# matsui528/rii

Measured on AMD Instinct MI355X. Metric: queries/sec, higher is better.
Workload: dtype f32; 1 GPU; SIFT1M-shaped linear search, D=128 M=32 Ks=256, N=1000000, batch=1024 per GPU, topk=1; global_batch=1024, lut_mode=exact, simd_order=avx512, scan_mode=8-bit filter + exact fp32 re-rank

## Files before the change

rii_amd/csrc/engine.hip:

```cpp
#include "rii_amd.h"
#include "rii_internal.h"

#include <algorithm>
#include <chrono>
#include <cmath>
#include <cstdarg>
#include <cstdio>
#include <cstring>
#include <map>
#include <mutex>
#include <numeric>
#include <random>
#include <string>
#include <thread>
#include <vector>

#define RII_API extern "C" __attribute__((visibility("default")))

using namespace riiamd;

static thread_local std::string g_err;
static int set_err(int code, const char *fmt, ...)
{
    char buf[1024];
// ... 133 lines not shown
    int timing = 0;
    hipStream_t stream = nullptr;
    int n_cu = 256;

    std::vector<float> codewords;
    std::vector<uint8_t> codes;
    std::vector<uint8_t> centers;
    std::vector<std::vector<int32_t>> lists;
    int64_t N = 0;

    DevBuf d_codewords, d_cnorm, d_codes, d_centers, d_symtab, d_pl_off, d_pl_ids, d_list_len;
    DevBuf d_lcodes; bool lcodes_valid = false;
    bool lcodes_failed = false, rot_failed = false;
    DevBuf d_rcent, d_rlcodes, d_rl_toff; bool rot_valid = false;
    int64_t quad_launches = 0;
    int64_t rot_launches = 0;
    DevBuf d_scan_codes, d_scan_perm;
    DevBuf d_fcodes;

    int64_t fc_cov = 0;
    int scan_order = 1;
    int scan_mx = 1;
    int slice_topk = 1;
    int host_spin = 1;
    bool ivf_q_host = false;
    unsigned int *spin_flag = nullptr;
    unsigned int spin_seq = 0;
    bool spin_used = false;
    int64_t spin_nflags = 0;
    int host_zero_copy = 1;
    int fused_rerank = 0;
    int small_topk = 1;
    int scan_pipe = 1;
    int scan_dual = 1;
    int64_t scan_cov = 0;
    int64_t scan_N = -1;
    bool have_symtab = false, have_cnorm = false, lists_dirty = true;


    std::map<std::string, KernelTimer> timers;
    std::vector<hipEvent_t> event_pool;

    ScratchSet parked;
    int lanes = 2;
    mutable std::mutex mu;

};

namespace {

int64_t nlist_of(const rii_engine *e) { return e->M ? (int64_t) (e->centers.size() / (size_t) e->M) : 0; }

bool timer_wanted(const rii_engine *e, const char *name)
{
    if (e->timing == 1) return true;
    if (e->timing == 2) return !strcmp(name, "scan") || !strcmp(name, "ivf_fused") || !strcmp(name, "ivf_scan") || !strcmp(name, "ivf_shard") || !strcmp(name, "shard_coarse");
    return false;
}
hipEvent_t timer_event(rii_engine *e)
{
    if (!e->event_pool.empty()) {
        hipEvent_t ev = e->event_pool.back();
        e->event_pool.pop_back();
        return ev;
    }
    hipEvent_t ev = nullptr;
// ... 268 lines not shown
        }
        HIP_TRY(launch_lut_build_mfma(d_queries, B, e->d_codewords.as<float>(), e->d_cnorm.as<float>(), e->M, e->Ks,
                                      e->Ds, qt, e->s_lut.as<float>(), st));
    } else {
        HIP_TRY(launch_lut_build(d_queries, B, e->d_codewords.as<float>(), e->M, e->Ks, e->Ds, e->arch, qt,
                                 e->s_lut.as<float>(), st));
    }
    return RII_OK;
}

int exact_tile_for(const rii_engine *e, int64_t B, int topk) { return (topk == 1 && B <= 2 && e->QT >= (int) B) ? (int) B : e->QT; }

void pick_chunks(const rii_engine *e, int64_t n_codes, int64_t B, int *chunks, int64_t *chunk_len, int qt = 0)
{
    if (qt <= 0) qt = e->QT;
    const int64_t tiles = (B + qt - 1) / qt;
    int64_t c = e->scan_chunks;
    if (c <= 0) {
        const bool stream_form = qt <= 2 && (size_t) qt * e->M * e->Ks * sizeof(float) <= ((size_t) 64 << 10);
        const int64_t target = (stream_form ? 4LL : 2LL) * e->n_cu;
        c = (target + tiles - 1) / tiles;
        const int64_t max_c = std::max<int64_t>(1, n_codes / 8192);
        c = std::max<int64_t>(1, std::min(c, max_c));
        if (tiles >= e->n_cu) c = 1;
    }
    c = std::max<int64_t>(1, std::min<int64_t>(c, 65535));
    int64_t len = (n_codes + c - 1) / c;
    len = std::max<int64_t>(len, 1);
    *chunks = (int) ((n_codes + len - 1) / len);
    *chunk_len = len;
}

constexpr int64_t kScanOrderMinN = 1 << 16;

int ensure_scan_order(rii_engine *e, hipStream_t st)
{
    if (e->scan_N == e->N) return RII_OK;
    const size_t M = (size_t) e->M;
    const int64_t cov = std::min(e->scan_cov, e->N);
    RII_TRY(e->d_scan_codes.ensure((size_t) e->N * M, (size_t) cov * M, st));
    RII_TRY(e->d_scan_perm.ensure((size_t) e->N * sizeof(int32_t), (size_t) cov * sizeof(int32_t), st));
    {
        ScopedTimer t(e, "scan_order", st);
        HIP_TRY(launch_scan_order(e->d_codes.as<uint8_t>(), e->N, e->M, e->Ks, fastscan_rows(e->M, e->Ks), cov / 1024,
                                  e->d_scan_perm.as<int32_t>(),
                                  e->d_scan_codes.as<uint8_t>(), st));
    }
    e->scan_cov = (e->N / 1024) * 1024;
    e->scan_N = e->N;
    HIP_TRY(hipStreamSynchronize(st));
    return RII_OK;
}

int ensure_fcodes(rii_engine *e, hipStream_t st)
{
    if (e->fc_cov == e->N) return RII_OK;
    RII_TRY(e->d_fcodes.ensure((size_t) fcodes_bytes(e->N, e->M, e->scan_mx), (size_t) fcodes_bytes(e->fc_cov, e->M, e->scan_mx), st));
    {
        ScopedTimer t(e, "format", st);
        HIP_TRY(launch_fcodes_format(e->d_codes.as<uint8_t>(), nullptr, e->fc_cov, e->N, e->M, e->Ks, e->d_fcodes.as<uint16_t>(),
                                     e->scan_mx, st));
    }
    e->fc_cov = e->N;
    HIP_TRY(hipStreamSynchronize(st));
    return RII_OK;
}
// ... 150 lines not shown
            if (!e->qlut_ready) {
                ScopedTimer t(e, "quant", st);
                RII_TRY(e->s_qc.ensure((size_t) B * e->M * e->Ks));
                const int lv = generic_table_levels(e);
                HIP_TRY(launch_lut_quantize(e->s_lut.as<float>(), B, e->M, e->Ks, e->lut_qt, e->s_qc.as<uint8_t>(),
                                            e->s_qlut.as<uint8_t>(), e->s_slack.as<int32_t>(), e->scan_mx, st, lv));
                e->qlut_levels = lv;
            }
            if (!e->qlut_ready) HIP_TRY(hipMemsetAsync(e->s_cand_cnt.p, 0, (size_t) B * sizeof(unsigned int), st));
            e->last_fs_B = B;
            if (topk == 1) {
                RII_TRY(e->s_gthr.ensure((size_t) B * sizeof(uint32_t)));
                if (!e->qlut_ready)
                    HIP_TRY(hipMemsetAsync(e->s_gthr.p, 0xff, (size_t) B * sizeof(uint32_t), st));
                const bool tail_rr = !e->lut_valid && e->fused_rerank && !d_perm && fscan_tail_supported(e->M, e->Ks, e->Ds, e->scan_mx);
                FsTail tl;
                if (tail_rr) {
                    RII_TRY(ensure_tile_done(e, st));
                    tl.queries = d_queries; tl.codewords = e->d_codewords.as<float>(); tl.codes = d_rr; tl.remap = d_remap;
                    tl.indirect = indirect; tl.Ds = e->Ds; tl.topk = topk; tl.out_ids = d_out_ids; tl.out_dists = d_out_dists;
                    tl.tile_done = e->s_tile_done.as<unsigned int>();
                    const int64_t nfl = fscan_tail_flags(e->M, e->Ks, e->scan_mx, e->scan_dual, B);
                    if (e->spin_flag && nfl * sizeof(unsigned int) <= kPinFlagWords * sizeof(unsigned int)) {
                        tl.host_flag = e->spin_flag; tl.seq = e->spin_seq;
                        e->spin_used = true; e->spin_nflags = nfl;
                    }
                }
                {
                    ScopedTimer t(e, "scan", st, true);
                    HIP_TRY(launch_fscan(d_scan, n_codes, e->M, e->Ks, e->s_qlut.as<uint8_t>(), e->s_slack.as<int32_t>(),
                                         (int) B, chunks, len, e->s_cand.as<unsigned long long>(),
                                         e->s_cand_cnt.as<unsigned int>(), cap, 0, nullptr, nullptr,
                                         e->s_gthr.as<uint32_t>(), 1, e->scan_mx, st, e->qlut_quarter ? 1 : 0, e->scan_dual, e->qlut_levels,
                                         tail_rr ? &tl : nullptr, e->scan_pipe == 2 || (e->scan_pipe == 1 && B <= 128)));
                }
                if (tail_rr) return RII_OK;
                ScopedTimer t(e, "rerank", st);
                if (!e->lut_valid) {
                    HIP_TRY(launch_rerank_top1_direct(d_rr, n_codes, e->M, e->Ds, d_queries, e->d_codewords.as<float>(),
                                                      e->s_slack.as<int32_t>(), e->s_cand.as<unsigned long long>(),
                                                      e->s_cand_cnt.as<unsigned int>(), cap, d_remap, B, d_out_ids, d_out_dists, topk,
                                                      indirect, st));
                    return RII_OK;
                }
                HIP_TRY(launch_rerank_top1(d_rr, n_codes, e->M, e->Ks, e->s_lut.as<float>(), e->lut_qt,
                                           e->s_slack.as<int32_t>(), e->s_cand.as<unsigned long long>(),
                                           e->s_cand_cnt.as<unsigned int>(), cap, d_remap, d_perm, B, d_out_ids, d_out_dists, topk,
                                           indirect, st, e->d_cand_peak.as<unsigned int>()));
                if (e->h_cand_peak && e->d_cand_peak.p)
                    HIP_TRY(hipMemcpyAsync(e->h_cand_peak, e->d_cand_peak.p, sizeof(unsigned int), hipMemcpyDeviceToHost, st));
                return RII_OK;
            }
            RII_TRY(e->s_segmin.ensure((size_t) B * G * sizeof(uint16_t)));
            RII_TRY(e->s_thr16.ensure((size_t) B * sizeof(uint32_t)));
            {
                ScopedTimer t(e, "scan", st, true);
                HIP_TRY(launch_fscan(d_scan, n_codes, e->M, e->Ks, e->s_qlut.as<uint8_t>(), e->s_slack.as<int32_t>(), (int) B,
                                     chunks, len, nullptr, nullptr, 0, 1, e->s_segmin.as<uint16_t>(), nullptr, nullptr, stride,
                                     e->scan_mx, st, e->qlut_quarter ? 1 : 0, e->scan_dual, e->qlut_levels));
            }
            {
                ScopedTimer t(e, "kth", st);
                HIP_TRY(launch_kth_threshold(e->s_segmin.as<uint16_t>(), G, B, topk, fastscan_max_sum(e->M, e->qlut_levels),
                                             e->s_slack.as<int32_t>(), e->s_thr16.as<uint32_t>(), st));
            }
            {
                ScopedTimer t(e, "scan", st, true);
// ... 1957 lines not shown
        e->shard_pre = (int) value;
    } else if (k == "ivf_quad") {
        e->ivf_quad = value < 0 ? 0 : (int) std::min<int64_t>(value, 2);
    } else if (k == "ivf_rot") {
        e->ivf_rot = value < 0 ? 0 : (int) std::min<int64_t>(value, 2);
        e->rot_failed = false;
        if (!value) { e->d_rcent.release(); e->d_rlcodes.release(); e->d_rl_toff.release(); e->rot_valid = false; }
    } else if (k == "ivf_inline_exact") {
        e->ivf_inline_exact = value ? 1 : 0;
    } else if (k == "ivf_list_codes") {
        e->ivf_list_codes = value ? 1 : 0;
        e->lcodes_failed = false; e->rot_failed = false;
        if (!value) { e->d_lcodes.release(); e->lcodes_valid = false; e->d_rlcodes.release(); e->rot_valid = false; }
    } else if (k == "ivf_force_exact") {
        e->ivf_force_exact = value ? 1 : 0;
    } else if (k == "fused_tables") {
        e->fused_tables = value ? 1 : 0;
    } else if (k == "generic_table_levels") {
        if (value != 0 && value != 63 && value != 127 && value != 255) return set_err(RII_ERR_INVALID, "generic_table_levels must be 0, 63, 127 or 255");
        e->generic_levels = (int) value;
    } else if (k == "table_levels") {
        if (value != 63 && value != 127 && value != 255) return set_err(RII_ERR_INVALID, "table_levels must be 63, 127 or 255");
        e->table_levels = (int) value;
    } else if (k == "scan_order") {
        e->scan_order = value ? 1 : 0;
    } else if (k == "scan_mx") {
        HIP_TRY(hipSetDevice(e->device));
        RII_TRY(begin_exclusive(e));
        e->scan_mx = value ? 1 : 0;
        e->fc_cov = 0;
    } else if (k == "scan_pipe") {
        if (value < 0 || value > 2) return set_err(RII_ERR_INVALID, "scan_pipe must be 0 (never), 1 (batches <= 128) or 2 (always)");
        e->scan_pipe = (int) value;
    } else if (k == "scan_dual") {
        e->scan_dual = value ? 1 : 0;
    } else if (k == "slice_topk") {
        e->slice_topk = value ? 1 : 0;
    } else if (k == "host_spin") {
        e->host_spin = value ? 1 : 0;
    } else if (k == "small_topk") {
        e->small_topk = value ? 1 : 0;
    } else if (k == "host_zero_copy") {
        if (value < 0 || value > 2) return set_err(RII_ERR_INVALID, "host_zero_copy must be 0 (never), 1 (auto) or 2 (always)");
        e->host_zero_copy = (int) value;
    } else if (k == "fused_rerank") {
        e->fused_rerank = value ? 1 : 0;
    } else if (k == "lanes") {
        if (value != 1 && value != 2) return set_err(RII_ERR_INVALID, "lanes must be 1 or 2");
        HIP_TRY(hipSetDevice(e->device));
        RII_TRY(begin_exclusive(e));
        e->lanes = (int) value;
    } else if (k == "fast_min_batch") {
        e->fast_min_batch = (int) std::max<int64_t>(0, value);
    } else if (k == "cand_cap") {
        if (value < 1 || value > (1 << 20)) return set_err(RII_ERR_INVALID, "bad cand_cap");
        e->cand_cap = (int) value;
        e->cand_cap_forced = true;
    } else {
        return set_err(RII_ERR_INVALID, "unknown option '%s'", key);
    }
    return RII_OK;
}
RII_API int64_t rii_get_option(const rii_engine *e, const char *key)
{
    if (!e || !key) return -1;
    std::lock_guard<std::mutex> guard(e->mu);
    const std::string k(key);
    if (k == "lut_mode") return e->lut_mode;
    if (k == "scan_chunks") return e->scan_chunks;
    if (k == "timing") return e->timing;
    if (k == "scan_mode") return e->scan_mode;
    if (k == "cand_cap") return e->cand_cap;
    if (k == "ivf_fused") return e->ivf_fused;
    if (k == "ivf_force_exact") return e->ivf_force_exact;
    if (k == "ivf_inline_exact") return e->ivf_inline_exact;
    if (k == "ivf_quad") return e->ivf_quad;
    if (k == "ivf_rot") return e->ivf_rot;
    if (k == "ivf_rot_launches") return e->rot_launches;
    if (k == "ivf_quad_launches") return e->quad_launches;
    if (k == "shard_pre_launches") return e->shard_pre_launches;
    if (k == "shard_pre") return e->shard_pre;
    if (k == "ivf_list_codes") return e->ivf_list_codes;
    if (k == "fused_tables") return e->fused_tables;
    if (k == "table_levels") return e->table_levels;
    if (k == "generic_table_levels") return e->generic_levels;
    if (k == "scan_order") return e->scan_order;
    if (k == "lanes") return e->lanes;
    if (k == "scan_mx") return e->scan_mx;
    if (k == "scan_dual") return e->scan_dual;
    if (k == "scan_pipe") return e->scan_pipe;
    if (k == "small_topk") return e->small_topk;
    if (k == "fused_rerank") return e->fused_rerank;
    if (k == "host_zero_copy") return e->host_zero_copy;
    if (k == "host_spin") return e->host_spin;
    if (k == "slice_topk") return e->slice_topk;
    if (k == "fast_min_batch") return e->fast_min_batch;
    if (k == "cand_total" || k == "cand_max") {
        if (e->last_fs_B == 0 || !e->s_cand_cnt.p) return 0;
        std::vector<unsigned int> h((size_t) e->last_fs_B);
        if (hipDeviceSynchronize() != hipSuccess) return -1;
        if (hipMemcpy(h.data(), e->s_cand_cnt.p, h.size() * sizeof(unsigned int), hipMemcpyDeviceToHost) != hipSuccess) return -1;
        int64_t tot = 0, mx = 0;
        for (unsigned int v : h) { tot += v; mx = std::max<int64_t>(mx, v); }
        return k == "cand_total" ? tot : mx;
    }
    if (k == "lut_tile") return e->QT;
    if (k == "n_cu") return e->n_cu;
    return -1;
}

RII_API int rii_timing_read(rii_engine *e, const char *kernel, double *total_ms, int64_t *launches)
{
    if (!e || !kernel) return set_err(RII_ERR_INVALID, "bad arguments");
    std::lock_guard<std::mutex> guard(e->mu);
    HIP_TRY(hipSetDevice(e->device));
    RII_TRY(begin_exclusive(e));
    KernelTimer &t = e->timers[kernel];
    for (auto &pr : t.pending) {
        HIP_TRY(hipEventSynchronize(pr.second));
        float ms = 0.f;
        HIP_TRY(hipEventElapsedTime(&ms, pr.first, pr.second));
        t.total_ms += ms;
        t.launches += 1;
// ... 30 lines not shown
```

rii_amd/csrc/fastscan.hip:

```cpp
#include "rii_internal.h"
#include "rii_device.h"
#include <float.h>
#include <algorithm>
#include <type_traits>

namespace riiamd {

constexpr int kFsThreads = 1024;
constexpr size_t kFsLdsBytes = 160 * 1024 - 512;
int fastscan_rows(int M, int Ks);
#ifndef RII_FS_LEVELS
#define RII_FS_LEVELS 63
#endif
constexpr int kFsLevels = RII_FS_LEVELS;
constexpr int kFsFlush = 255 / kFsLevels;
static_assert(kFsFlush * kFsLevels <= 255 && (kFsFlush == 4 || kFsFlush == 8), "byte-packed partial sums must not carry");

template <typename Getter>
__device__ __forceinline__ void quantize_table(const Getter &T, int64_t b, int M, int Ks,
                                               uint8_t *__restrict__ qc, int32_t *__restrict__ slack, int levels = kFsLevels)
{
    __shared__ float s_lo[256], s_hi[256];
    __shared__ double s_rlo[256], s_rhi[256];
    __shared__ float s_delta;
// ... 2111 lines not shown
        }
        __syncthreads();
        for (int q = tid >> 6; q < QR; q += kFsThreads >> 6) {
            const int b = tile * QR + q;
            const unsigned int c = min(s_lcnt[q], (unsigned int) p.lcap), base = s_lcnt[QR + q];
            for (unsigned int i = tid & 63; i < c; i += 64)
                if (base + i < (unsigned int) p.cap) {
                    if constexpr (TAIL) fs_cand_store(&p.cand[(size_t) b * p.cap + base + i], s_lcand[(size_t) q * p.lcap + i]);
                    else p.cand[(size_t) b * p.cap + base + i] = s_lcand[(size_t) q * p.lcap + i];
                }
        }
    }
    if constexpr (TAIL) {
        fs_kernarg_t pa = (fs_kernarg_t) __builtin_amdgcn_kernarg_segment_ptr();
        asm volatile("" : "+s"(pa));
        bool spilled = false;
        for (int q = 0; q < 16; ++q) spilled |= s_lcnt[q] > (uint32_t) pa->lcap;
        if (fs_tail_arrive(pa, s_lcnt, tid, spilled)) {
            if (pa->tail.Ds == 4) fs_tail_rerank<float4, 16>(pa, tile * 16, smem, tid);
            else fs_tail_rerank<float2, 16>(pa, tile * 16, smem, tid);
        }
    }
    if constexpr (MODE == 1) {
        const size_t G = (size_t) gridDim.x * kFsMxSeg;
        const size_t seg = (size_t) blockIdx.x * kFsMxSeg + wave * 16 + col;
#pragma unroll
        for (int r = 0; r < 4; ++r) {
            const int b = tile * QR + 4 * gq + r;
            if (4 * gq + r < QR && b < p.B) p.segmin[(size_t) b * G + seg] = (uint16_t) (keep[r] > 0xffff ? 0xffff : keep[r]);
        }
    }
}

__device__ __forceinline__ void fs_mx_issue_hot_dual(uint32_t w, const uint32_t (&C)[8], v4i_t (&r)[8])
{
    fs_mx_issue2<0>(w, C[0], C[1], r[0], r[1]);
    fs_mx_issue2<2>(w, C[2], C[3], r[2], r[3]);
    fs_mx_issue2<0>(w, C[4], C[5], r[4], r[5]);
    fs_mx_issue2<2>(w, C[6], C[7], r[6], r[7]);
}
__device__ __forceinline__ void fs_mx_reduce_refill_dual(v4i_t (&r)[8], uint32_t wn, const uint32_t (&C)[8], const v4i_t &spa, int spidx,
                                                         const v4i_t &zero, v4i_t &accA, v4i_t &accB)
{
    accA = fs_acc_init(zero);
    {
        const v8i_t b = __builtin_shufflevector(r[0], r[1], 0, 1, 2, 3, 4, 5, 6, 7);
        accA = __builtin_amdgcn_smfmac_i32_16x16x128_i8(spa, b, accA, spidx, 0, 0);
        fs_mx_issue2<0>(wn, C[0], C[1], r[0], r[1]);
    }
    {
        const v8i_t b = __builtin_shufflevector(r[2], r[3], 0, 1, 2, 3, 4, 5, 6, 7);
        accA = __builtin_amdgcn_smfmac_i32_16x16x128_i8(spa, b, accA, spidx, 0, 0);
        fs_mx_issue2<2>(wn, C[2], C[3], r[2], r[3]);
    }
    accB = fs_acc_init(zero);
    {
        const v8i_t b = __builtin_shufflevector(r[4], r[5], 0, 1, 2, 3, 4, 5, 6, 7);
        accB = __builtin_amdgcn_smfmac_i32_16x16x128_i8(spa, b, accB, spidx, 0, 0);
        fs_mx_issue2<0>(wn, C[4], C[5], r[4], r[5]);
    }
    {
        const v8i_t b = __builtin_shufflevector(r[6], r[7], 0, 1, 2, 3, 4, 5, 6, 7);
        accB = __builtin_amdgcn_smfmac_i32_16x16x128_i8(spa, b, accB, spidx, 0, 0);
        fs_mx_issue2<2>(wn, C[6], C[7], r[6], r[7]);
    }
}
// ... 281 lines not shown
            if (bB < p.B) p.segmin[(size_t) bB * G + seg] = (uint16_t) (keepB[r] > 0xffff ? 0xffff : keepB[r]);
        }
    }
}

template <int MODE, bool TAIL = false> static hipError_t launch_fscan_mx_dual_t(const FsArgs &a, int chunks, hipStream_t st)
{
    const size_t tab = (size_t) 2 * 16 * 256 * 16 + 32 * 4 + 32 * 8 + 32 * 4;
    FsArgs b = a;
    b.lcap = (MODE != 0) ? 0 : (int) std::min<size_t>(128, (kFsLdsBytes - tab) / ((size_t) 32 * 8));
    size_t smem = tab + (size_t) 32 * 8 * b.lcap;
    if (TAIL) smem = std::max(smem, kFsTailLds);
    auto kern = fscan_mx_dual_kernel<MODE, TAIL>;
    hipError_t e = hipFuncSetAttribute(reinterpret_cast<const void *>(kern), hipFuncAttributeMaxDynamicSharedMemorySize, (int) smem);
    if (e != hipSuccess) return e;
    launch_timed(kern, dim3(chunks, (a.B + 31) / 32), dim3(kFsThreads), smem, st, b);
    return hipGetLastError();
}

template <int T, int MODE, int QR = 16, bool TAIL = false, bool PIPE = false> static hipError_t launch_fscan_mx_t(const FsArgs &a, int chunks, int tiles, hipStream_t st)
{
    const size_t tab = (size_t) a.M * a.Ks * QR + 64 + (size_t) QR * 8 + 64;
    FsArgs b = a;
    b.lcap = (MODE != 0) ? 0 : (int) std::min<size_t>(128, (kFsLdsBytes - tab) / ((size_t) QR * 8));
    size_t smem = tab + (size_t) QR * 8 * b.lcap;
    if (TAIL) smem = std::max(smem, kFsTailLds);
    auto kern = fscan_mx_kernel<T, MODE, QR, TAIL, PIPE>;
    hipError_t e = hipFuncSetAttribute(reinterpret_cast<const void *>(kern), hipFuncAttributeMaxDynamicSharedMemorySize, (int) smem);
    if (e != hipSuccess) return e;
    launch_timed(kern, dim3(chunks, tiles), dim3(kFsThreads), smem, st, b);
    return hipGetLastError();
}

template <int MODE> static hipError_t launch_fscan_mode(const FsArgs &a, int chunks, bool rot, bool mx, hipStream_t st)
{
    const int qr = fastscan_rows(a.M, a.Ks);
    const int tiles = (a.B + qr - 1) / qr;
    if (rot && mx) {
        if constexpr (MODE == 0) {
            if (a.tail.queries) {
                if (a.M == 16 && a.dual) return launch_fscan_mx_dual_t<0, true>(a, chunks, st);
                if (a.M == 16) return launch_fscan_mx_t<4, 0, 16, true>(a, chunks, tiles, st);
                if (a.M == 32) return launch_fscan_mx_t<8, 0, 16, true>(a, chunks, tiles, st);
                return hipErrorInvalidValue;
            }
            if (a.bias == 0 && a.pipe) {
                if (a.M == 16 && !a.dual) return launch_fscan_mx_t<4, 0, 16, false, true>(a, chunks, tiles, st);
                if (a.M == 32) return launch_fscan_mx_t<8, 0, 16, false, true>(a, chunks, tiles, st);
            }
        }
        if (a.M == 16 && a.dual) return launch_fscan_mx_dual_t<MODE>(a, chunks, st);
        if (a.M == 16) return launch_fscan_mx_t<4, MODE>(a, chunks, tiles, st);
        if (a.M == 32) return launch_fscan_mx_t<8, MODE>(a, chunks, tiles, st);
        if (a.M == 64) return launch_fscan_mx_t<16, MODE, 8>(a, chunks, tiles, st);
        return hipErrorInvalidValue;
    }
    if (rot) {
        if (qr == 16 && a.M == 16) return launch_fscan_t<4, 256, MODE, 16, true>(a, chunks, tiles, st);
        if (qr == 16 && a.M == 32) return launch_fscan_t<8, 256, MODE, 16, true>(a, chunks, tiles, st);
        return hipErrorInvalidValue;
    }
    if (qr == 16) {
        if (a.Ks == 256 && a.M == 8) return launch_fscan_t<2, 256, MODE, 16>(a, chunks, tiles, st);
        if (a.Ks == 256 && a.M == 16) return launch_fscan_t<4, 256, MODE, 16>(a, chunks, tiles, st);
        if (a.Ks == 256 && a.M == 32) return launch_fscan_t<8, 256, MODE, 16>(a, chunks, tiles, st);
        return launch_fscan_t<0, 0, MODE, 16>(a, chunks, tiles, st);
    }
    if (a.Ks == 256 && a.M == 64) return launch_fscan_t<16, 256, MODE, 8>(a, chunks, tiles, st);
    return launch_fscan_t<0, 0, MODE, 8>(a, chunks, tiles, st);
}

hipError_t launch_fscan(const uint8_t *d_codes, int64_t n_codes, int M, int Ks, const uint8_t *d_qlut,
                        const int32_t *d_slack, int B, int chunks, int64_t chunk_len, unsigned long long *d_cand,
                        unsigned int *d_cand_count, int cap, int mode, uint16_t *d_segmin, const uint32_t *d_thr16,
                        uint32_t *d_gthr, int sample_stride, int mx, hipStream_t st, int quarter, int dual, int levels, const FsTail *tail, int pipe)
{
    if (B == 0 || n_codes == 0) return hipSuccess;
    const bool rot = fs_rot_supported(M, Ks, mx);
    FsArgs a;
    a.quarter = quarter;
    a.dual = ((dual & 1) && mx && M == 16 && rot) ? 1 : 0;
    a.bias = levels > 127 ? 128 * M : 0;
    a.pipe = pipe;
    if (tail && tail->queries) {
        if (mode != 0 || !fscan_tail_supported(M, Ks, tail->Ds, mx)) return hipErrorInvalidValue;
        a.tail = *tail;
    }
    a.gthr = d_gthr;
    a.sample_stride = sample_stride < 1 ? 1 : sample_stride;
    a.codes = d_codes; a.n_codes = n_codes; a.M = M; a.Ks = Ks; a.qlut = d_qlut; a.slack = d_slack; a.B = B;
    a.chunk_len = chunk_len; a.cand = d_cand; a.cand_count = d_cand_count; a.cap = cap; a.segmin = d_segmin;
    a.thr16 = d_thr16;
    if (mode == 1) return launch_fscan_mode<1>(a, chunks, rot, mx != 0, st);
    if (mode == 2) return launch_fscan_mode<2>(a, chunks, rot, mx != 0, st);
    return launch_fscan_mode<0>(a, chunks, rot, mx != 0, st);
}

bool fscan_tail_supported(int M, int Ks, int Ds, int mx)
{
    return mx && Ks == 256 && (M == 16 || M == 32) && (Ds == 4 || Ds == 2) && fs_rot_supported(M, Ks, mx);
}
int fscan_tail_flags(int M, int Ks, int mx, int dual, int64_t B)
{
    const int qpb = fscan_queries_per_block(M, Ks, mx, dual);
    return (int) ((B + qpb - 1) / qpb);
}
int fscan_queries_per_block(int M, int Ks, int mx, int dual)
{
    return (dual && mx && M == 16 && fs_rot_supported(M, Ks, mx)) ? 32 : fastscan_rows(M, Ks);
}
int fscan_mx_subspace(int M, int lane, int t)
{
    return M == 64 ? fs_mx_subspace64(lane >> 4, lane & 15, t) : fs_mx_subspace(lane >> 4, lane & 15, t);
}
int fscan_segments_per_chunk(int M, int Ks, int mx) { return (mx && fs_rot_supported(M, Ks, mx)) ? kFsMxSeg : kFsThreads; }
int64_t fcodes_bytes(int64_t n, int M, int mx) { return mx ? (n + 15) / 16 * 16 * M : n * M * 2;
}

__global__ __launch_bounds__(256) void kth_threshold_kernel(const uint16_t *__restrict__ segmin, int64_t G, int k,
                                                            int maxv, const int32_t *__restrict__ slack,
                                                            uint32_t *__restrict__ thr16)
{
    extern __shared__ __attribute__((aligned(16))) unsigned char smem[];
    int *hist = reinterpret_cast<int *>(smem);
    __shared__ int s_part[256];
// ... 409 lines not shown
```

rii_amd/csrc/rii_internal.h:

```cpp
#pragma once
#include <hip/hip_runtime.h>
#include <hip/hip_ext.h>
#include <stdint.h>
#include <stddef.h>

namespace riiamd {

struct LaunchEvents {
    hipEvent_t start = nullptr, stop = nullptr;
};
extern thread_local LaunchEvents g_launch_events;
template <typename K, typename A>
inline void launch_timed(K kern, dim3 grid, dim3 block, size_t smem, hipStream_t st, const A &arg)
{
    if (g_launch_events.start && g_launch_events.stop) {
        hipExtLaunchKernelGGL(kern, grid, block, (uint32_t) smem, st, g_launch_events.start, g_launch_events.stop, 0, arg);
        g_launch_events = LaunchEvents();
    } else {
        hipLaunchKernelGGL(kern, grid, block, smem, st, arg);
    }
}


constexpr int kScanThreads = 1024;
// ... 108 lines not shown
                           int Ks, uint8_t *d_centers, hipStream_t st);

hipError_t segmented_sort_keys(unsigned long long *d_keys_in, unsigned long long *d_keys_out, int64_t segs,
                               int64_t len, void **d_temp, size_t *temp_bytes, hipStream_t st);

int lut_tile_for(int M, int Ks);

bool fastscan_supported(int M, int Ks);
int fastscan_rows(int M, int Ks);
hipError_t launch_lut_quantize(const float *d_lut, int64_t B, int M, int Ks, int QT, uint8_t *d_qc, uint8_t *d_qlut,
                               int32_t *d_slack, int mx, hipStream_t st, int levels = 63);
hipError_t launch_lut_build_quant(const float *d_queries, int64_t B, const float *d_codewords, int M, int Ks, int Ds,
                                  int arch, float *d_lut, uint8_t *d_qc, uint8_t *d_qlut, int32_t *d_slack,
                                  unsigned int *d_cand_cnt, uint32_t *d_gthr, int mx, hipStream_t st, int levels = 63);
bool fs_rot_supported(int M, int Ks, int mx);
struct FsTail {
    const float *queries = nullptr;
    const float *codewords = nullptr;
    const uint8_t *codes = nullptr;
    const int64_t *remap = nullptr;
    int indirect = 0, Ds = 4, topk = 1;
    int64_t *out_ids = nullptr;
    float *out_dists = nullptr;
    unsigned int *tile_done = nullptr;
    unsigned int *host_flag = nullptr;
    unsigned int seq = 0;
};
bool fscan_tail_supported(int M, int Ks, int Ds, int mx);
int fscan_tail_flags(int M, int Ks, int mx, int dual, int64_t B);
hipError_t launch_fscan(const uint8_t *d_codes, int64_t n_codes, int M, int Ks, const uint8_t *d_qlut,
                        const int32_t *d_slack, int B, int chunks, int64_t chunk_len, unsigned long long *d_cand,
                        unsigned int *d_cand_count, int cap, int mode, uint16_t *d_segmin, const uint32_t *d_thr16,
                        uint32_t *d_gthr, int sample_stride, int mx, hipStream_t st, int quarter = 0, int dual = 0, int levels = 63,
                        const FsTail *tail = nullptr, int pipe = 1);
int fscan_queries_per_block(int M, int Ks, int mx, int dual);
int fastscan_max_sum(int M, int levels = 0);
bool qlut_fused_supported(int M, int Ks, int Ds, int mx);
size_t qlut_fused_bytes(int64_t B, int M);
hipError_t launch_qlut_fused(const float *d_queries, int64_t B, const float *d_codewords, int M, int Ds, float *d_lut_or_null,
                             uint32_t *d_qlut4, int32_t *d_slack, unsigned int *d_cand_cnt, uint32_t *d_gthr, int levels, hipStream_t st);
bool rerank_direct_supported(int M, int Ks, int Ds);
hipError_t launch_rerank_top1_direct(const uint8_t *d_codes, int64_t n_codes, int M, int Ds, const float *d_queries,
                                     const float *d_codewords, const int32_t *d_slack, const unsigned long long *d_cand,
                                     const unsigned int *d_cand_count, int cap, const int64_t *d_remap, int64_t B,
                                     int64_t *d_out_ids, float *d_out_dists, int topk, int indirect, hipStream_t st);
int fscan_segments_per_chunk(int M, int Ks, int mx);
int fscan_mx_subspace(int M, int lane, int t);
int64_t fcodes_bytes(int64_t n, int M, int mx);
bool lut_tile_supported(int M, int Ks, int Ds, int mx);
hipError_t launch_lut_tile_build_quant(const float *d_queries, int64_t B, const float *d_codewords, int M, int Ds, float *d_lut,
                                       float *d_lohi, uint8_t *d_qlut, int32_t *d_slack, unsigned int *d_cand_cnt,
                                       uint32_t *d_gthr, hipStream_t st);
bool fs_rot_supported(int M, int Ks, int mx);
hipError_t launch_fcodes_format(const uint8_t *d_codes, const int64_t *d_ids, int64_t n0, int64_t n1, int M, int Ks,
                                uint16_t *d_out, int mx, hipStream_t st);
int rerank_topk_max_k();
hipError_t launch_kth_threshold(const uint16_t *d_segmin, int64_t G, int64_t B, int k, int maxv, const int32_t *d_slack,
                                uint32_t *d_thr16, hipStream_t st);
hipError_t launch_rerank_topk(const uint8_t *d_codes, int64_t n_codes, int M, int Ks, const float *d_lut, int QT,
                              const unsigned long long *d_cand, const unsigned int *d_cand_count, int cap,
                              const int64_t *d_remap, const int32_t *d_perm, int64_t B, int64_t *d_out_ids,
                              float *d_out_dists, int topk, int32_t *d_flag_list, int *d_nflag, int indirect, hipStream_t st);
hipError_t launch_rerank_top1(const uint8_t *d_codes, int64_t n_codes, int M, int Ks, const float *d_lut, int QT,
                              const int32_t *d_slack, const unsigned long long *d_cand,
                              const unsigned int *d_cand_count, int cap, const int64_t *d_remap,
                              const int32_t *d_perm, int64_t B, int64_t *d_out_ids, float *d_out_dists, int topk,
                              int indirect, hipStream_t st, unsigned int *d_peak = nullptr);
// ... 109 lines not shown
```

Before: 3.003 million queries/s.

## Add cascade fastscan kernel that scores half the subspaces before full evaluation

Adds a new M=32 matrix-core fast-scan kernel that first accumulates distances over the first half of subspaces. It finishes the remaining subspaces only when some lane in the wave has a partial sum below its query threshold. Survivors are staged in LDS and flushed to the global candidate list in bulk. The kernel is selected by default for batches above 128 with at least 2^18 codes. It trades fewer matrix ops and fewer code-byte reads on rejected groups for extra branching, and it relies on partial sums being a valid lower bound.

```diff
diff --git a/rii_amd/csrc/engine.hip b/rii_amd/csrc/engine.hip
--- a/rii_amd/csrc/engine.hip
+++ b/rii_amd/csrc/engine.hip
@@ -189,6 +189,7 @@
     int fused_rerank = 0;
     int small_topk = 1;
     int scan_pipe = 1;
+    int scan_cascade = 1;
     int scan_dual = 1;
     int64_t scan_cov = 0;
     int64_t scan_N = -1;
@@ -523,6 +524,7 @@
 }
 
 constexpr int64_t kScanOrderMinN = 1 << 16;
+constexpr int64_t kCascadeMinCodes = 1 << 18;
 
 int ensure_scan_order(rii_engine *e, hipStream_t st)
 {
@@ -739,7 +741,8 @@
                                          (int) B, chunks, len, e->s_cand.as<unsigned long long>(),
                                          e->s_cand_cnt.as<unsigned int>(), cap, 0, nullptr, nullptr,
                                          e->s_gthr.as<uint32_t>(), 1, e->scan_mx, st, e->qlut_quarter ? 1 : 0, e->scan_dual, e->qlut_levels,
-                                         tail_rr ? &tl : nullptr, e->scan_pipe == 2 || (e->scan_pipe == 1 && B <= 128)));
+                                         tail_rr ? &tl : nullptr, e->scan_pipe == 2 || (e->scan_pipe == 1 && B <= 128),
+                                         e->scan_cascade == 2 || (e->scan_cascade == 1 && B > 128 && n_codes >= kCascadeMinCodes)));
                 }
                 if (tail_rr) return RII_OK;
                 ScopedTimer t(e, "rerank", st);
@@ -2763,6 +2766,9 @@
     } else if (k == "scan_pipe") {
         if (value < 0 || value > 2) return set_err(RII_ERR_INVALID, "scan_pipe must be 0 (never), 1 (batches <= 128) or 2 (always)");
         e->scan_pipe = (int) value;
+    } else if (k == "scan_cascade") {
+        if (value < 0 || value > 2) return set_err(RII_ERR_INVALID, "scan_cascade must be 0 (never), 1 (batches > 128, scans >= 2^18 codes) or 2 (always)");
+        e->scan_cascade = (int) value;
     } else if (k == "scan_dual") {
         e->scan_dual = value ? 1 : 0;
     } else if (k == "slice_topk") {
@@ -2820,6 +2826,7 @@
     if (k == "scan_mx") return e->scan_mx;
     if (k == "scan_dual") return e->scan_dual;
     if (k == "scan_pipe") return e->scan_pipe;
+    if (k == "scan_cascade") return e->scan_cascade;
     if (k == "small_topk") return e->small_topk;
     if (k == "fused_rerank") return e->fused_rerank;
     if (k == "host_zero_copy") return e->host_zero_copy;
diff --git a/rii_amd/csrc/fastscan.hip b/rii_amd/csrc/fastscan.hip
--- a/rii_amd/csrc/fastscan.hip
+++ b/rii_amd/csrc/fastscan.hip
@@ -2167,6 +2167,240 @@
     }
 }
 
+__global__ __launch_bounds__(kFsThreads) void fscan_mx_kernel_cascade(FsArgs p)
+{
+    constexpr int T = 8, M = 32, QR = 16;
+    typedef typename FsMxW<T>::V W;
+    extern __shared__ __attribute__((aligned(16))) unsigned char smem[];
+    const int tid = threadIdx.x, tile = blockIdx.y;
+    constexpr size_t lut_bytes = (size_t) M * 256 * QR;
+    uint32_t *s_thr = reinterpret_cast<uint32_t *>(smem + lut_bytes);
+    uint32_t *s_lcnt = reinterpret_cast<uint32_t *>(smem + lut_bytes + 64);
+    uint32_t *s_slk = reinterpret_cast<uint32_t *>(smem + lut_bytes + 64 + QR * 8);
+    unsigned long long *s_lcand = reinterpret_cast<unsigned long long *>(smem + lut_bytes + 64 + QR * 8 + 64);
+    {
+        if (tid < 16) s_slk[tid] = (tile * QR + tid < p.B) ? (uint32_t) p.slack[tile * QR + tid] : 0u;
+        if (p.quarter) {
+            const uint32_t *src = reinterpret_cast<const uint32_t *>(p.qlut) + (size_t) tile * 4 * M * 256;
+            const int slot = tid & 15, qq = (tid >> 4) & 3;
+            for (int unit = tid >> 6; unit < M; unit += kFsThreads >> 6) {
+                const int h = unit >> 4, ks0 = (unit & 15) * 16;
+                const uint4 *sp = reinterpret_cast<const uint4 *>(src + ((size_t) qq * M + 16 * h + slot) * 256 + ks0);
+                const uint4 v0 = sp[0], v1 = sp[1], v2 = sp[2], v3 = sp[3];
+                uint32_t *d = reinterpret_cast<uint32_t *>(smem + ((size_t) h * 4096 + (size_t) ks0 * 16 + slot) * 16 + qq * 4);
+                d[0 * 64] = v0.x; d[1 * 64] = v0.y; d[2 * 64] = v0.z; d[3 * 64] = v0.w;
+                d[4 * 64] = v1.x; d[5 * 64] = v1.y; d[6 * 64] = v1.z; d[7 * 64] = v1.w;
+                d[8 * 64] = v2.x; d[9 * 64] = v2.y; d[10 * 64] = v2.z; d[11 * 64] = v2.w;
+                d[12 * 64] = v3.x; d[13 * 64] = v3.y; d[14 * 64] = v3.z; d[15 * 64] = v3.w;
+            }
+        } else {
+            const uint4 *s4 = reinterpret_cast<const uint4 *>(p.qlut + (size_t) tile * lut_bytes);
+            uint4 *d4 = reinterpret_cast<uint4 *>(smem);
+            for (size_t i = tid; i < lut_bytes / 16; i += kFsThreads) d4[i] = s4[i];
+        }
+        if (tid < 16) s_thr[tid] = (tile * QR + tid < p.B) ? 0xffffu : 0u;
+        if (tid < 2 * QR) s_lcnt[tid] = 0u;
+    }
+    __syncthreads();
+    const int lane = tid & 63, wave = tid >> 6, col = lane & 15, gq = lane >> 4;
+    v4i_t spa;
+    int spidx;
+    fs_mx_pattern(col, spa, spidx);
+    uint32_t Ch[4];
+    fs_mx_consts<4>(lane, Ch);
+    auto lane_now = [&]() {
+        int l = lane;
+        asm volatile("" : "+v"(l));
+        return l;
+    };
+
+    const int64_t c_begin = (int64_t) blockIdx.x * p.chunk_len;
+    int64_t c_end = c_begin + p.chunk_len;
+    if (c_end > p.n_codes) c_end = p.n_codes;
+    const int64_t span = c_end > c_begin ? c_end - c_begin : 0;
+    const int full = (int) (span / kFsThreads);
+    const int tail_groups = (int) ((span - (int64_t) full * kFsThreads + 15) / 16);
+    const W *fc = reinterpret_cast<const W *>(p.codes) + (size_t) (c_begin / 16) * 64 + lane;
+
+    auto emit = [&](int q, uint32_t a, uint32_t t, uint32_t n) {
+        const int b = tile * QR + q;
+        if (b >= p.B) return;
+        const uint32_t nt = fs_thr_of(a, s_slk[q]);
+        if (nt < t) {
+            atomicMin(&s_thr[q], nt);
+            atomicMin(&p.gthr[b], nt);
+        }
+        const unsigned long long rec = ((unsigned long long) a << 32) | n;
+        bool staged = false;
+        if (p.lcap > 0) {
+            const unsigned int lp = atomicAdd(&s_lcnt[q], 1u);
+            if (lp < (unsigned int) p.lcap) { s_lcand[(size_t) q * p.lcap + lp] = rec; staged = true; }
+        }
+        if (!staged) {
+            const unsigned int pos = atomicAdd(&p.cand_count[b], 1u);
+            if (pos < (unsigned int) p.cap) p.cand[(size_t) b * p.cap + pos] = rec;
+        }
+    };
+    auto judge = [&](const v4i_t &acc, const v4i_t &thr, uint32_t n) {
+        const bool h0 = acc[0] < thr[0], h1 = acc[1] < thr[1], h2 = acc[2] < thr[2], h3 = acc[3] < thr[3];
+        if (h0 | h1 | h2 | h3) {
+            uint32_t mask = (h0 ? 1u : 0u) | (h1 ? 2u : 0u) | (h2 ? 4u : 0u) | (h3 ? 8u : 0u);
+            while (mask) {
+                const int r = __ffs((int) mask) - 1;
+                mask &= mask - 1u;
+                const int a = r == 0 ? acc[0] : r == 1 ? acc[1] : r == 2 ? acc[2] : acc[3];
+                const int t = r == 0 ? thr[0] : r == 1 ? thr[1] : r == 2 ? thr[2] : thr[3];
+                emit(4 * gq + r, (uint32_t) a, (uint32_t) t, n);
+            }
+        }
+    };
+    v4i_t keep = {0x7fffffff, 0x7fffffff, 0x7fffffff, 0x7fffffff};
+    auto take_min = [&](const v4i_t &acc) {
+#pragma unroll
+        for (int r = 0; r < 4; ++r) keep[r] = acc[r] < keep[r] ? acc[r] : keep[r];
+    };
+    auto publish = [&]() {
+#pragma unroll
+        for (int r = 0; r < 4; ++r) {
+            int v = keep[r];
+#pragma unroll
+            for (int off = 8; off > 0; off >>= 1) {
+                const int o = __shfl_xor(v, off);
+                v = o < v ? o : v;
+            }
+            const int b = tile * QR + 4 * gq + r;
+            if (col == 0 && v != 0x7fffffff && b < p.B) atomicMin(&s_thr[4 * gq + r], fs_thr_of((uint32_t) v, s_slk[4 * gq + r]));
+        }
+    };
+    auto load_thr = [&]() { return *reinterpret_cast<const v4i_t *>(s_thr + 4 * gq); };
+    auto adopt = [&](bool first) {
+        int q = tid;
+        asm volatile("" : "+v"(q));
+        if (q < QR) {
+            const int b = tile * QR + q;
+            if (b < p.B) {
+                const uint32_t g = __hip_atomic_load(&p.gthr[b], __ATOMIC_RELAXED, __HIP_MEMORY_SCOPE_AGENT);
+                if (first) {
+                    const uint32_t mine = s_thr[q];
+                    if (mine < g) atomicMin(&p.gthr[b], mine);
+                }
+                atomicMin(&s_thr[q], g);
+            }
+        }
+    };
+    auto slow_group = [&](int64_t gi, bool minima, const v4i_t &thr) {
+        const int l = lane_now();
+        const W w = (reinterpret_cast<const W *>(p.codes) + (size_t) (c_begin / 16) * 64 + l)[(size_t) gi * 64];
+        uint32_t C[T];
+        fs_mx_consts<T>(l, C);
+        v4i_t r[T];
+        fs_mx_issue<T>(w, C, r);
+        v4i_t acc = fs_mx_reduce<T>(r, spa, spidx);
+        const int64_t n = c_begin + gi * 16 + col;
+        if (n >= c_end) acc = v4i_t{0x7fffffff, 0x7fffffff, 0x7fffffff, 0x7fffffff};
+        if (minima) take_min(acc);
+        else judge(acc, thr, (uint32_t) n);
+    };
+    auto tail = [&](bool minima) {
+        const v4i_t thr = load_thr();
+        for (int gi = wave; gi < tail_groups; gi += kFsThreads / 64) slow_group((int64_t) full * 64 + gi, minima, thr);
+    };
+
+    if (full > 0) {
+        const v4i_t none = {0, 0, 0, 0};
+#pragma unroll 1
+        for (int j = 0; j < 4; ++j) slow_group(wave * 4 + j, true, none);
+    } else {
+        tail(true);
+    }
+    publish();
+    __syncthreads();
+    adopt(true);
+    __syncthreads();
+
+    const int ntrip = full;
+    auto trip_of = [&](int k) { return k + 1 < full ? k + 1 : 0; };
+    if (ntrip > 0) {
+        const W *pw = fc + (size_t) wave * 4 * 64;
+        auto trip_ptr = [&](int k) { return pw + (size_t) trip_of(k < ntrip ? k : ntrip - 1) * 64 * 64; };
+        constexpr int S = 64 * (int) sizeof(W);
+        v4i_t r0[4], r1[4], r2[4], r3[4];
+        W q[4];
+        uint32_t y[4];
+        {
+            const W *p0 = trip_ptr(0), *p1 = trip_ptr(1);
+            const W g0 = p0[0], g1 = p0[64], g2 = p0[128], g3 = p0[192];
+            fs_mx_issue_hot<4>(g0.x, Ch, r0);
+            fs_mx_issue_hot<4>(g1.x, Ch, r1);
+            fs_mx_issue_hot<4>(g2.x, Ch, r2);
+            fs_mx_issue_hot<4>(g3.x, Ch, r3);
+            y[0] = g0.y; y[1] = g1.y; y[2] = g2.y; y[3] = g3.y;
+            fs_mx_load<0>(q[0], p1);
+            fs_mx_load<S>(q[1], p1);
+            fs_mx_load<2 * S>(q[2], p1);
+            fs_mx_load<3 * S>(q[3], p1);
+        }
+        const uint32_t thr_addr = (uint32_t) (lut_bytes + 16 * gq);
+        v4i_t thr;
+        asm volatile("ds_read_b128 %0, %1\n\ts_waitcnt lgkmcnt(0)" : "=v"(thr) : "v"(thr_addr));
+        auto group = [&](v4i_t (&r)[4], W &qj, uint32_t &yj, const W *pnn, auto off, uint32_t n) {
+            constexpr int OFF = decltype(off)::value;
+            fs_mx_vmwait<3>(qj);
+            fs_mx_wait<13>(r);
+            v4i_t acc = fs_mx_reduce_refill<4, true>(r, qj.x, Ch, spa, spidx, spa);
+            const uint32_t yh = yj;
+            asm volatile("v_mov_b32 %1, %2\n\tglobal_load_dwordx2 %0, %3, off offset:%4" : "=v"(qj), "=&v"(yj) : "v"(qj.y), "v"(pnn), "n"(OFF));
+            const bool h = (acc[0] < thr[0]) | (acc[1] < thr[1]) | (acc[2] < thr[2]) | (acc[3] < thr[3]);
+            if (__builtin_amdgcn_ballot_w64(h)) {
+                uint32_t Cf[8];
+                fs_mx_consts<8>(lane_now(), Cf);
+                v4i_t f0, f1;
+                fs_mx_issue2<0>(yh, Cf[4], Cf[5], f0, f1);
+                fs_mx_wait<0>(r0); fs_mx_wait<0>(r1); fs_mx_wait<0>(r2); fs_mx_wait<0>(r3);
+                asm volatile("s_waitcnt lgkmcnt(0)" : "+v"(thr), "+v"(f0), "+v"(f1));
+                acc = __builtin_amdgcn_smfmac_i32_16x16x128_i8(spa, __builtin_shufflevector(f0, f1, 0, 1, 2, 3, 4, 5, 6, 7), acc, spidx, 0, 0);
+                fs_mx_issue2<2>(yh, Cf[6], Cf[7], f0, f1);
+                asm volatile("s_waitcnt lgkmcnt(0)" : "+v"(f0), "+v"(f1));
+                acc = __builtin_amdgcn_smfmac_i32_16x16x128_i8(spa, __builtin_shufflevector(f0, f1, 0, 1, 2, 3, 4, 5, 6, 7), acc, spidx, 0, 0);
+                judge(acc, thr, n);
+            }
+        };
+        for (int k = 0; k < ntrip; ++k) {
+            const int it = trip_of(k);
+            const W *pnn = trip_ptr(k + 2);
+            int t_ = tid;
+            asm volatile("" : "+v"(t_));
+            const uint32_t n = (uint32_t) c_begin + (uint32_t) it * kFsThreads + (uint32_t) (t_ & 0x3cf);
+            group(r0, q[0], y[0], pnn, std::integral_constant<int, 0>{}, n);
+            group(r1, q[1], y[1], pnn, std::integral_constant<int, S>{}, n + 16);
+            asm volatile("ds_read_b128 %0, %1 ; rii:inflight-ok (tools/check_isa_inflight.py)" : "+v"(thr) : "v"(thr_addr));
+            group(r2, q[2], y[2], pnn, std::integral_constant<int, 2 * S>{}, n + 32);
+            group(r3, q[3], y[3], pnn, std::integral_constant<int, 3 * S>{}, n + 48);
+            adopt(false);
+        }
+        fs_mx_wait<0>(r0); fs_mx_wait<0>(r1); fs_mx_wait<0>(r2); fs_mx_wait<0>(r3);
+        asm volatile("s_waitcnt lgkmcnt(0)" : "+v"(thr));
+        fs_mx_vmwait<0>(q[0]); fs_mx_vmwait<0>(q[1]); fs_mx_vmwait<0>(q[2]); fs_mx_vmwait<0>(q[3]);
+    }
+    tail(false);
+
+    if (p.lcap > 0) {
+        __syncthreads();
+        if (tid < QR) {
+            const int b = tile * QR + tid;
+            const unsigned int c = min(s_lcnt[tid], (unsigned int) p.lcap);
+            s_lcnt[QR + tid] = (c && b < p.B) ? atomicAdd(&p.cand_count[b], c) : 0u;
+        }
+        __syncthreads();
+        for (int q = tid >> 6; q < QR; q += kFsThreads >> 6) {
+            const int b = tile * QR + q;
+            const unsigned int c = min(s_lcnt[q], (unsigned int) p.lcap), base = s_lcnt[QR + q];
+            for (unsigned int i = tid & 63; i < c; i += 64)
+                if (base + i < (unsigned int) p.cap) p.cand[(size_t) b * p.cap + base + i] = s_lcand[(size_t) q * p.lcap + i];
+        }
+    }
+}
+
 __device__ __forceinline__ void fs_mx_issue_hot_dual(uint32_t w, const uint32_t (&C)[8], v4i_t (&r)[8])
 {
     fs_mx_issue2<0>(w, C[0], C[1], r[0], r[1]);
@@ -2514,6 +2748,18 @@
     return hipGetLastError();
 }
 
+static hipError_t launch_fscan_mx_cascade(const FsArgs &a, int chunks, int tiles, hipStream_t st)
+{
+    const size_t tab = (size_t) a.M * a.Ks * 16 + 64 + 16 * 8 + 64;
+    FsArgs b = a;
+    b.lcap = (int) std::min<size_t>(128, (kFsLdsBytes - tab) / (16 * 8));
+    const size_t smem = tab + 16 * 8 * (size_t) b.lcap;
+    hipError_t e = hipFuncSetAttribute(reinterpret_cast<const void *>(fscan_mx_kernel_cascade), hipFuncAttributeMaxDynamicSharedMemorySize, (int) smem);
+    if (e != hipSuccess) return e;
+    launch_timed(fscan_mx_kernel_cascade, dim3(chunks, tiles), dim3(kFsThreads), smem, st, b);
+    return hipGetLastError();
+}
+
 template <int MODE> static hipError_t launch_fscan_mode(const FsArgs &a, int chunks, bool rot, bool mx, hipStream_t st)
 {
     const int qr = fastscan_rows(a.M, a.Ks);
@@ -2555,7 +2801,7 @@
 hipError_t launch_fscan(const uint8_t *d_codes, int64_t n_codes, int M, int Ks, const uint8_t *d_qlut,
                         const int32_t *d_slack, int B, int chunks, int64_t chunk_len, unsigned long long *d_cand,
                         unsigned int *d_cand_count, int cap, int mode, uint16_t *d_segmin, const uint32_t *d_thr16,
-                        uint32_t *d_gthr, int sample_stride, int mx, hipStream_t st, int quarter, int dual, int levels, const FsTail *tail, int pipe)
+                        uint32_t *d_gthr, int sample_stride, int mx, hipStream_t st, int quarter, int dual, int levels, const FsTail *tail, int pipe, int cascade)
 {
     if (B == 0 || n_codes == 0) return hipSuccess;
     const bool rot = fs_rot_supported(M, Ks, mx);
@@ -2573,6 +2819,7 @@
     a.codes = d_codes; a.n_codes = n_codes; a.M = M; a.Ks = Ks; a.qlut = d_qlut; a.slack = d_slack; a.B = B;
     a.chunk_len = chunk_len; a.cand = d_cand; a.cand_count = d_cand_count; a.cap = cap; a.segmin = d_segmin;
     a.thr16 = d_thr16;
+    if (cascade && mode == 0 && rot && mx && M == 32 && a.bias == 0 && !a.tail.queries) return launch_fscan_mx_cascade(a, chunks, (B + 15) / 16, st);
     if (mode == 1) return launch_fscan_mode<1>(a, chunks, rot, mx != 0, st);
     if (mode == 2) return launch_fscan_mode<2>(a, chunks, rot, mx != 0, st);
     return launch_fscan_mode<0>(a, chunks, rot, mx != 0, st);
diff --git a/rii_amd/csrc/rii_internal.h b/rii_amd/csrc/rii_internal.h
--- a/rii_amd/csrc/rii_internal.h
+++ b/rii_amd/csrc/rii_internal.h
@@ -164,7 +164,7 @@
                         const int32_t *d_slack, int B, int chunks, int64_t chunk_len, unsigned long long *d_cand,
                         unsigned int *d_cand_count, int cap, int mode, uint16_t *d_segmin, const uint32_t *d_thr16,
                         uint32_t *d_gthr, int sample_stride, int mx, hipStream_t st, int quarter = 0, int dual = 0, int levels = 63,
-                        const FsTail *tail = nullptr, int pipe = 1);
+                        const FsTail *tail = nullptr, int pipe = 1, int cascade = 0);
 int fscan_queries_per_block(int M, int Ks, int mx, int dual);
 int fastscan_max_sum(int M, int levels = 0);
 bool qlut_fused_supported(int M, int Ks, int Ds, int mx);
```

After: 3.519 million queries/s, median of 6. +17.2%, better.
